# chonlei/neural-ode-ion-channels

Measured on AMD Instinct MI355X. Metric: trajectories/sec (sinewave protocol, 100k steps), higher is better.
Workload: dtype f64

## Files before the change

include/ionode.h:

```cpp
#ifndef IONODE_H
#define IONODE_H

#include <stddef.h>
#include <stdint.h>

#ifdef __cplusplus
extern "C" {
#endif

#define IONODE_ABI_VERSION 10

#define IONODE_MODEL_HH2 0
#define IONODE_MODEL_MARKOV6 1
#define IONODE_MODEL_NNF 2
#define IONODE_MODEL_NND 3

#define IONODE_STATUS_OK 0
#define IONODE_STATUS_DT_UNDERFLOW 1
#define IONODE_STATUS_NONFINITE 2
#define IONODE_STATUS_MAX_STEPS 3

#define IONODE_OK 0
#define IONODE_ERR_ARG (-1)
#define IONODE_ERR_UNSUPPORTED (-2)
// ... 25 lines not shown
  double t_eval_dt_hint;
  int64_t max_total_steps;
  double *ckpt;
  int32_t ckpt_cap;
  int32_t t_eval_exact;
  const double *sse_ref;
  double *sse_out;
  double max_step;
  const double *v_at_outputs;
  int64_t mlp_image_stride;
  int32_t traj_per_image;
  const int32_t *launch_order;
} ionode_desc;

#define IONODE_DEFAULT_MAX_TOTAL_STEPS 1000000

size_t ionode_mlp_packed_floats(int32_t mlp_layers, int32_t mlp_width);

int ionode_mlp_pack(const float *state_dict_flat, int32_t mlp_layers, int32_t mlp_width, float *packed);

int ionode_dopri5(const ionode_desc *d, const float *mlp_packed, const double *params, const double *prot_v,
                  const double *prot_t, const int32_t *prot_of_traj, const void *y0, const double *t_eval,
                  void *y_out, double *i_out, int32_t *status, int64_t *stats, void *stream);

int ionode_protocol_at_outputs(const ionode_desc *d, const double *prot_v, const double *prot_t, const double *t_eval,
                               double *v_out, void *stream);

int ionode_launch_geometry(const ionode_desc *d, int32_t out[4]);

const char *ionode_kernel_name(const ionode_desc *d);

const char *ionode_last_kernel_name(void);

int32_t ionode_lane_wise_from(int32_t model, int32_t mlp_width);

const char *ionode_last_error(void);
int32_t ionode_abi_version(void);


size_t ionode_grad_image_floats(int32_t mlp_layers, int32_t mlp_width);
int ionode_grad_pack(const float *state_dict_flat, int32_t mlp_layers, int32_t mlp_width, float *image);

size_t ionode_grad_record_floats(int32_t mlp_layers, int32_t mlp_width);

int ionode_dopri5_backward(const ionode_desc *d, int32_t it_begin, int32_t it_end, int32_t n_iter, const float *grad_image,
                           const double *params, const double *prot_v, const double *prot_t, const int32_t *prot_of_traj,
// ... 60 lines not shown
```

neural-ode-ion-channels_amd/capi.py:

```python
import ctypes as C
import os
import subprocess

import numpy as np
import torch

_HERE = os.path.dirname(os.path.abspath(__file__))
LIB_PATH = os.environ.get("IONODE_LIB") or os.path.join(_HERE, "libionode.so")

MODEL_HH2, MODEL_MARKOV6, MODEL_NNF, MODEL_NND = 0, 1, 2, 3
STATUS_OK, STATUS_DT_UNDERFLOW, STATUS_NONFINITE, STATUS_MAX_STEPS = 0, 1, 2, 3
STATUS_TEXT = {
    0: "ok",
    1: "underflow in dt",
    2: "non-finite values in state `y`",
    3: "max_num_steps exceeded",
}
ABI_VERSION = 10

EXPORTS = (
    "ionode_abi_version", "ionode_last_error", "ionode_mlp_packed_floats", "ionode_mlp_pack",
    "ionode_launch_geometry", "ionode_kernel_name", "ionode_last_kernel_name", "ionode_lane_wise_from", "ionode_dopri5", "ionode_protocol_at_outputs",
    "ionode_grad_image_floats", "ionode_grad_pack", "ionode_grad_record_floats", "ionode_dopri5_backward", "ionode_dopri5_backward_sse",
    "ionode_grad_packet_doubles", "ionode_dopri5_backward_recompute", "ionode_dopri5_backward_sweep",
    "ionode_dopri5_backward_sse_gc", "ionode_dopri5_backward_recompute_sse", "ionode_dopri5_backward_sweep_sse",
    "ionode_grad_partial_floats", "ionode_grad_reduce", "ionode_grad_reduce_unit", "ionode_grad_reduce_slabs", "ionode_grad_last_error",
    "ionode_regress_step", "ionode_adam_step", "ionode_image_refresh", "ionode_regress_plan",
)

SWEEP_BUFFERS = {
    "ionode_dopri5_backward": ("grad_image", "params", "prot_v", "prot_t", "prot_of_traj", "t_eval", "n_accepted", "grad_y", "state",
                               "records", "grad_params", "grad_y0"),
    "ionode_dopri5_backward_sse": ("params", "prot_v", "prot_t", "prot_of_traj", "t_eval", "n_accepted", "grad_sse", "state",
                                   "grad_params", "grad_y0"),
    "ionode_dopri5_backward_recompute": ("grad_image", "params", "prot_v", "prot_t", "prot_of_traj", "t_eval", "n_accepted", "grad_y",
                                         "records", "packets"),
    "ionode_dopri5_backward_sweep": ("grad_image", "params", "prot_v", "prot_t", "prot_of_traj", "t_eval", "n_accepted", "grad_y", "state",
                                     "records", "packets", "grad_params", "grad_y0"),
    "ionode_dopri5_backward_sse_gc": ("prot_v", "prot_t", "prot_of_traj", "t_eval", "n_accepted", "grad_sse", "packets", "sse_grad_y0"),
    "ionode_dopri5_backward_recompute_sse": ("grad_image", "params", "prot_v", "prot_t", "prot_of_traj", "t_eval", "n_accepted", "records",
                                             "packets"),
    "ionode_dopri5_backward_sweep_sse": ("grad_image", "params", "prot_v", "prot_t", "prot_of_traj", "t_eval", "n_accepted", "sse_grad_y0",
                                         "state", "records", "packets", "grad_params", "grad_y0"),
}


def n_state(model):
    return 6 if model == MODEL_MARKOV6 else 2


# ... 35 lines not shown

_lib = None


def lib():
    global _lib
    if _lib is None:
        if not os.path.exists(LIB_PATH):
            raise IonodeError(f"{LIB_PATH} is missing: run `python -c 'import __graft_entry__ as g; g.build()'` "
                              "(there is no CPU fallback for the integrator)")
        L = C.CDLL(LIB_PATH)
        L.ionode_abi_version.restype = C.c_int32
        L.ionode_last_error.restype = C.c_char_p
        L.ionode_kernel_name.restype = C.c_char_p
        L.ionode_kernel_name.argtypes = [C.POINTER(IonodeDesc)]
        L.ionode_mlp_packed_floats.restype = C.c_size_t
        L.ionode_mlp_packed_floats.argtypes = [C.c_int32, C.c_int32]
        L.ionode_mlp_pack.restype = C.c_int
        L.ionode_mlp_pack.argtypes = [C.c_void_p, C.c_int32, C.c_int32, C.c_void_p]
        L.ionode_launch_geometry.restype = C.c_int
        L.ionode_launch_geometry.argtypes = [C.POINTER(IonodeDesc), C.POINTER(C.c_int32 * 4)]
        L.ionode_dopri5.restype = C.c_int
        L.ionode_dopri5.argtypes = [C.POINTER(IonodeDesc)] + [C.c_void_p] * 12
        L.ionode_grad_last_error.restype = C.c_char_p
        for fn in (L.ionode_grad_image_floats, L.ionode_grad_record_floats, L.ionode_grad_partial_floats):
            fn.restype = C.c_size_t
            fn.argtypes = [C.c_int32, C.c_int32]
        L.ionode_grad_pack.restype = C.c_int
        L.ionode_grad_pack.argtypes = [C.c_void_p, C.c_int32, C.c_int32, C.c_void_p]
        L.ionode_grad_packet_doubles.restype = C.c_size_t
        L.ionode_grad_packet_doubles.argtypes = []
        for name, buffers in SWEEP_BUFFERS.items():
            getattr(L, name).restype = C.c_int
            getattr(L, name).argtypes = [C.POINTER(IonodeDesc), C.c_int32, C.c_int32, C.c_int32] + [C.c_void_p] * (len(buffers) + 1)
        L.ionode_grad_reduce.restype = C.c_int
        L.ionode_grad_reduce.argtypes = [C.c_int32, C.c_int32, C.c_void_p, C.c_int64, C.c_int32, C.c_void_p, C.c_void_p]
        L.ionode_grad_reduce_slabs.restype = C.c_int32
        L.ionode_grad_reduce_slabs.argtypes = [C.c_int32, C.c_int32, C.c_int64]
        L.ionode_grad_reduce_unit.restype = C.c_int
        L.ionode_grad_reduce_unit.argtypes = [C.c_int32, C.c_int32, C.c_void_p, C.c_int64, C.c_int32, C.c_void_p, C.c_void_p]
        L.ionode_regress_step.restype = C.c_int
        L.ionode_regress_step.argtypes = [C.c_int32, C.c_int32, C.c_void_p, C.c_void_p, C.c_void_p, C.c_void_p, C.c_int32,
                                          C.c_float, C.c_void_p, C.c_void_p, C.c_int32, C.c_void_p]
        L.ionode_regress_plan.restype = C.c_int
        L.ionode_regress_plan.argtypes = [C.c_int32, C.c_int32, C.POINTER(C.c_int32 * 3)]
        L.ionode_adam_step.restype = C.c_int
# ... 40 lines not shown
    return h.hexdigest()


def make_desc(**kw):
    d = IonodeDesc()
    for k, v in kw.items():
        setattr(d, k, v)
    return d


def launch_geometry(desc):
    out = (C.c_int32 * 4)()
    rc = lib().ionode_launch_geometry(C.byref(desc), C.byref(out))
    if rc != 0:
        raise IonodeError(last_error())
    return {"grid": out[0], "block": out[1], "lds_bytes": out[2], "tile_waves": out[3]}


def regress_plan(mlp_layers, mlp_width):
    out = (C.c_int32 * 3)()
    if lib().ionode_regress_plan(int(mlp_layers), int(mlp_width), C.byref(out)) != 0:
        raise IonodeError(lib().ionode_grad_last_error().decode())
    return {"generic": bool(out[0]), "wg_per_cu": out[1], "lds_bytes": out[2]}


def kernel_name(desc):
    return lib().ionode_kernel_name(C.byref(desc)).decode()


def _dev_ptr(t, dtype, name, shape=None):
    if t is None:
        return None
    if not isinstance(t, torch.Tensor) or not t.is_cuda:
        raise IonodeError(f"{name}: expected a CUDA/HIP tensor (the integrator has no CPU path)")
    if t.dtype != dtype or not t.is_contiguous():
        raise IonodeError(f"{name}: expected contiguous {dtype}, got {t.dtype} contiguous={t.is_contiguous()}")
    if shape is not None and tuple(t.shape) != tuple(shape):
        raise IonodeError(f"{name}: expected shape {tuple(shape)}, got {tuple(t.shape)}")
    return C.c_void_p(t.data_ptr())


_order_cache = {}


def _protocol_major(prot_of_traj):
    key = (prot_of_traj.data_ptr(), prot_of_traj._version, int(prot_of_traj.shape[0]), str(prot_of_traj.device))
# ... 78 lines not shown
        desc.sse_ref, desc.sse_out = sse_ref.data_ptr(), sse.data_ptr()
    elif not states:
        raise IonodeError("states=False needs sse_ref (something must be computed)")
    i_out = out.get("i")
    if current and i_out is None:
        i_out = torch.empty((B, Nt), dtype=torch.float64, device=dev)
    status = out.get("status")
    if status is None:
        status = torch.empty((B,), dtype=torch.int32, device=dev)
    st = out.get("stats")
    if stats and st is None:
        st = torch.empty((B, 4), dtype=torch.int64, device=dev)
    s = stream if stream is not None else torch.cuda.current_stream(dev).cuda_stream
    vtab = None
    if (current or sse_ref is not None) and model in (MODEL_HH2, MODEL_MARKOV6) and v_at_outputs is not None:
        if isinstance(v_at_outputs, str):
            if 4 * P <= B:
                vtab = protocol_at_outputs(desc, prot_v, prot_t, t_eval, stream=s)
        else:
            vtab = v_at_outputs
            _dev_ptr(vtab, torch.float64, "v_at_outputs", (P, Nt))
        if vtab is not None:
            desc.v_at_outputs = vtab.data_ptr()
    rc = lib().ionode_dopri5(
        C.byref(desc),
        _dev_ptr(mlp_packed, torch.float32, "mlp_packed"),
        _dev_ptr(params, torch.float64, "params", (B, params.shape[1])),
        _dev_ptr(prot_v, torch.float64, "prot_v"),
        _dev_ptr(prot_t, torch.float64, "prot_t", (Np,)) if prot_t is not None else None,
        _dev_ptr(prot_of_traj, torch.int32, "prot_of_traj", (B,)) if prot_of_traj is not None else None,
        _dev_ptr(y0, sdt, "y0"),
        _dev_ptr(t_eval, torch.float64, "t_eval"),
        _dev_ptr(y, sdt, "y_out", (B, Nt, D)) if y is not None else None,
        _dev_ptr(i_out, torch.float64, "i_out", (B, Nt)) if i_out is not None else None,
        _dev_ptr(status, torch.int32, "status", (B,)),
        _dev_ptr(st, torch.int64, "stats", (B, 4)) if st is not None else None,
        C.c_void_p(s),
    )
    if rc != 0:
        raise IonodeError(f"ionode_dopri5 failed ({rc}): {last_error()}")
    return {"y": y, "i": i_out, "status": status, "stats": st, "sse": sse, "desc": desc, "v_at_outputs": vtab,
            "kernel": lib().ionode_last_kernel_name().decode()}


def uniform_grid(t_eval):
    n = int(t_eval.shape[0])
    if n < 2:
        return None
    t0 = t_eval[0]
    dt = (t_eval[n - 1] - t0) / (n - 1)
    dev = (t_eval - (t0 + torch.arange(n, dtype=torch.float64, device=t_eval.device) * dt)).abs().max()
    t0, dt, dev = (float(x) for x in torch.stack([t0, dt, dev]).cpu())
    return (t0, dt, dev) if dt > 0 and dev <= 0.5 * dt else None


def sweep_launch(name, desc, it_begin, it_end, n_iter, stream, **buffers):
    names = SWEEP_BUFFERS[name]
    if set(buffers) != set(names):
        raise TypeError(f"{name}: missing {sorted(set(names) - set(buffers))}, unknown {sorted(set(buffers) - set(names))}")
    ptrs = [None if buffers[n] is None else C.c_void_p(buffers[n].data_ptr()) for n in names]
# ... 15 lines not shown
```

neural-ode-ion-channels_amd/csrc/ionode_attempt_body.hpp:

```cpp
#ifdef IONODE_STAMPS
    constexpr int NET = std::is_same<typename std::decay<decltype(IONODE_NET)>::type, MlpShrink4>::value ? 1 : 0;
    const unsigned long long att0_ = stamp_now();
#endif
    if constexpr (LW) {
#pragma unroll
      for (int i = 0; i < NPAR; ++i) asm volatile("" : "+v"(p[i]));
    }
    bool failed_now = false;
    if (active) {
      if ((int64_t)since >= a.max_steps || (int64_t)nacc + nrej >= a.max_total) { status = IONODE_STATUS_MAX_STEPS; failed_now = true; }
      else if (!(t + dt > t)) { status = IONODE_STATUS_DT_UNDERFLOW; failed_now = true; }
      else {
        bool fin = true;
#pragma unroll
        for (int d = 0; d < D; ++d) fin = fin && isfinite((double)y[d]);
        if (!fin) { status = IONODE_STATUS_NONFINITE; failed_now = true; }
      }
      if (failed_now) active = false;
    }
    {
      unsigned long long fm = __ballot(failed_now && lane < LPS);
      while (fm) {
        const int jj = __builtin_ctzll(fm);
        fm &= fm - 1;
// ... 140 lines not shown
      }
    }
    STAMP(stamps_, 8);
    if (LEAN || LEANM || a.te_dt > 0.0) {
      int n_out = 0;
      if (acc_now) {
        const double gf = floor((t1 - a.te_t0) * a.te_rdt);
        long long g = (gf < (double)(oi - 1)) ? (long long)(oi - 1) : ((gf > (double)(Nt - 1)) ? (long long)(Nt - 1) : (long long)gf);
        if ((LW && LEAN && D > 2) || (!LW && a.te_exact)) {
          while (g >= oi && te_at((int)g) > t1) --g;
          while (g + 1 < Nt && te_at((int)g + 1) <= t1) ++g;
        } else {
          while (g >= oi && a.t_eval[g] > t1) --g;
          while (g + 1 < Nt && a.t_eval[g + 1] <= t1) ++g;
        }
        n_out = (int)(g - oi + 1);
      }
      STAMP(stamps_, 9);
      if constexpr (!LW && G > 1) {
      constexpr int NS = (LPS >= WPS) ? LPS / WPS : 1;
      const bool exact = a.te_exact != 0;
      const bool want_i = (a.i_out != nullptr) || (a.sse_out != nullptr);
      const bool ugrid = a.prot_t == nullptr;
      int o_[NS], n_[NS], ip_[NS];
      double tk_[NS], plo_[NS], phi_[NS];
      bool inr_[NS];
      const double *pv_[NS];
#pragma unroll
      for (int k = 0; k < NS; ++k) {
        const int jj = wis + WPS * k;
        o_[k] = __builtin_amdgcn_readlane(oi, jj);
        n_[k] = (LPS >= WPS || jj < LPS) ? __builtin_amdgcn_readlane(n_out, jj) : 0;
        pv_[k] = a.prot_v + (size_t)__builtin_amdgcn_readlane(pidx, jj) * a.Np;
        tk_[k] = 0.0;
        if (lane < n_[k]) tk_[k] = exact ? te_at(o_[k] + lane) : a.t_eval[o_[k] + lane];
      }
      if (want_i && ugrid) {
#pragma unroll
        for (int k = 0; k < NS; ++k) {
          inr_[k] = protocol_index(a, tk_[k], ip_[k]);
          plo_[k] = pv_[k][ip_[k] - 1]; phi_[k] = pv_[k][ip_[k]];
        }
      }
      STAMP(stamps_, 10);
#pragma unroll
      for (int k = 0; k < NS; ++k) {
        const int jj = wis + WPS * k;
        const int n = n_[k], o = o_[k];
        if (n > 0) {
          const double t0b = bcast_f64(t0, jj), denb = bcast_f64(den, jj), rdenb = bcast_f64(rden, jj);
          S cb[5][D];
#pragma unroll
          for (int c = 0; c < 5; ++c)
#pragma unroll
            for (int d = 0; d < D; ++d) cb[c][d] = bcast<S>(ic[c][d], jj);
// ... 18 lines not shown
#pragma unroll
                for (int d = 0; d < D; ++d) out[d] = out[d] + xp * cb[c][d];
              }
              if (yo) store_state<S, D>(yo + (size_t)idx * D, out);
              if (want_i) {
                double vk;
                if (c0 == 0 && ugrid) vk = inr_[k] ? protocol_from(a, plo_[k], phi_[k], ip_[k], tk) : a.v_oob;
                else protocol_v(a, pv_[k], tk, vk);
                S gate;
                if (a.obs_open) gate = out[D - 1]; else gate = out[0] * out[1];
                if (a.obs_g != 1.0) gate = (S)a.obs_g * gate;
                const double ik = (double)gate * (vk - a.obs_e);
                if (io) io[idx] = ik;
                if (refb) { const double rr = ik - refb[idx]; sacc += rr * rr; }
              }
            }
          }
          if (a.sse_out) {
#pragma unroll
            for (int msk = 32; msk >= 1; msk >>= 1) sacc += __shfl_xor(sacc, msk);
            if (j == jj) sse += sacc;
          }
        }
      }
      oi += n_out;
      } else {
      bool packed_lane = false;
      if constexpr (LW && (VTAB || D > 2 || (CF2 && F::lean == Lean::States))) {
        constexpr int PK = 8, PKL = (D == 2) ? 4 : 2, NSL = PK / PKL;
        typedef S SV __attribute__((ext_vector_type(NSL)));
        const bool want_i = (a.i_out != nullptr) || (a.sse_out != nullptr);
        if (a.te_exact && (VTAB ? (want_i && (D > 2 || a.y_out == nullptr)) : (!want_i && a.y_out != nullptr))) {
          int lane_e = lane;
          asm volatile("" : "+v"(lane_e));
          packed_lane = n_out > 0 && lane_e < LPS && n_out <= 64;
          const unsigned long long emd = __ballot(packed_lane);
          auto emit_packed = [&](auto wi_tag) {
            constexpr bool WI = decltype(wi_tag)::value;
            const int nch = (n_out + PK - 1) / PK;
            if (packed_lane) *reinterpret_cast<int2 *>(lsm + lane_e * ROWB + 24) = make_int2(oi, oi + n_out);
            const int x = nch - 1;
            const unsigned long long m0 = __ballot(packed_lane && (x & 1)), m1 = __ballot(packed_lane && (x & 2)), m2 = __ballot(packed_lane && (x & 4));
            const int q = mbcnt(m0, mbcnt(emd)) + 2 * mbcnt(m1) + 4 * mbcnt(m2);
            const int C = __builtin_popcountll(emd) + __builtin_popcountll(m0) + 2 * __builtin_popcountll(m1) + 4 * __builtin_popcountll(m2);
#pragma unroll
            for (int i = 0; i < 8; ++i)
// ... 312 lines not shown
```

neural-ode-ion-channels_amd/csrc/ionode_capi.hip:

```cpp
#include <algorithm>
#include <cstdio>
#include <cstdlib>
#include <cstring>
#include <vector>

#include "ionode_launch.hpp"

namespace {

constexpr int kTile32From = 8192;
constexpr int kTile4Upto = 1024;
constexpr int kTile1Upto = 256;
constexpr int kTiny64From = 32769;
constexpr int kHh2LaneFrom = 49152;
constexpr int kMarkov6LaneFrom = 24576;

thread_local char g_err[256] = "";
thread_local const char *g_last_kernel = "";

void set_err(const char *fmt, const char *detail = "") { snprintf(g_err, sizeof g_err, fmt, detail); }

inline int np_of(int N) { return 16 * ((N + 15) / 16); }

struct Plan {
// ... 108 lines not shown
  if (!pl->v) {
    set_err("MLP width outside the compiled kernel variants: 1 <= N <= 512 (tuned tiles for N = 10, 100, 200, 500 -- architectures "
            "s00-s11 -- and the run-time-width tile for every other N; tile_waves must be 0 or 4 for the latter)");
    return IONODE_ERR_UNSUPPORTED;
  }
  const ionode::Variant *v = pl->v;
  const size_t tiles = (size_t)((d->n_traj + v->traj_per_tile - 1) / v->traj_per_tile);
  pl->grid = (unsigned)tiles;
  pl->block = 64u * v->G;
  pl->lds = v->lds_bytes(L, NT);
  if (v->shrink) {
    const char *ts = getenv("IONODE_TILE_SHRINK");
    pl->tile_shrink = ts == nullptr || ts[0] == '\0' || atoi(ts) != 0;
    pl->lds = std::max(pl->lds, ionode::MlpTile4::lds_bytes(L));
  }
  if (v->lane_wise) plan_lane_wise(pl, tiles, ((pl->lds + 15) & ~(size_t)15) + (size_t)ionode::LwLds::bytes(2, v->lds_key));
  if (d->traj_per_image > 0) {
    if (d->traj_per_image % v->traj_per_tile != 0 || d->mlp_image_stride < (int64_t)ionode_mlp_packed_floats(L, d->mlp_width)) {
      set_err("traj_per_image must be a multiple of the tile size (16; 64 with tile_waves = 64; 32 with tile_waves = 8) and mlp_image_stride at least one packed image");
      return IONODE_ERR_ARG;
    }
  }
  return IONODE_OK;
}

int make_plan(const ionode_desc *d, Plan *pl, bool want_current = false, bool explicit_grid = false) {
  if (!d) { set_err("null descriptor"); return IONODE_ERR_ARG; }
#ifdef IONODE_STAMPS
  const bool has_step_log = false;
#else
  const bool has_step_log = d->step_log != nullptr;
#endif
  const bool mlp = d->model == IONODE_MODEL_NNF || d->model == IONODE_MODEL_NND;
  const int D = d->model == IONODE_MODEL_MARKOV6 ? 6 : 2;
  if (d->model < 0 || d->model > 3) { set_err("unknown model"); return IONODE_ERR_ARG; }
  if (d->n_state != D) { set_err("n_state does not match model"); return IONODE_ERR_ARG; }
  if (d->n_traj < 1 || d->n_out < 1 || d->n_prot < 1 || d->prot_n < 2) { set_err("empty batch / grid / protocol"); return IONODE_ERR_ARG; }
  if (d->n_params < (D == 6 ? 12 : 8)) { set_err("n_params too small for model"); return IONODE_ERR_ARG; }
  if (!(d->rtol > 0) || !(d->atol >= 0) || !(d->prot_dt > 0)) { set_err("rtol/atol/prot_dt must be positive"); return IONODE_ERR_ARG; }
  const Ask k = {want_current, explicit_grid, has_step_log};
  return mlp ? plan_mlp(d, pl, k) : plan_closed(d, pl, k, D);
}

}

namespace ionode {
// ... 225 lines not shown
}

int ionode_launch_geometry(const ionode_desc *d, int32_t out[4]) {
  Plan pl;
  const int rc = make_plan(d, &pl);
  if (rc != IONODE_OK) return rc;
  out[0] = (int32_t)pl.grid;
  out[1] = (int32_t)pl.block;
  out[2] = (int32_t)pl.lds;
  out[3] = pl.v->G;
  return IONODE_OK;
}

const char *ionode_kernel_name(const ionode_desc *d) {
  Plan pl;
  if (make_plan(d, &pl, d && (d->sse_out != nullptr || d->v_at_outputs != nullptr)) != IONODE_OK) return "";
  return pl.v->name;
}

const char *ionode_last_kernel_name(void) { return g_last_kernel; }

int32_t ionode_lane_wise_from(int32_t model, int32_t mlp_width) { return lane_wise_from(model, mlp_width); }

int ionode_dopri5(const ionode_desc *d, const float *mlp_packed, const double *params, const double *prot_v,
                  const double *prot_t, const int32_t *prot_of_traj, const void *y0, const double *t_eval,
                  void *y_out, double *i_out, int32_t *status, int64_t *stats, void *stream) {
  Plan pl;
  const int rc = make_plan(d, &pl, i_out != nullptr || d->sse_out != nullptr, prot_t != nullptr);
  if (rc != IONODE_OK) return rc;
  const bool mlp = d->model == IONODE_MODEL_NNF || d->model == IONODE_MODEL_NND;
  if (!params || !prot_v || !y0 || !t_eval || (!y_out && !d->sse_out) || !status || (mlp && !mlp_packed)) {
    set_err("ionode_dopri5: required buffer is NULL");
    return IONODE_ERR_ARG;
  }
  if (d->sse_out && (!d->sse_ref || !(d->t_eval_dt_hint > 0.0) || d->n_out < 2)) {
    set_err("fused objective: sse_out needs sse_ref and the output-grid hint (t_eval_dt_hint > 0)");
    return IONODE_ERR_ARG;
  }
  ionode::KArgs a;
  memset(&a, 0, sizeof a);
  a.mlp = mlp_packed; a.params = params; a.prot_v = prot_v; a.prot_t = prot_t; a.prot_of_traj = prot_of_traj;
  a.y0 = y0; a.t_eval = t_eval; a.y_out = y_out; a.i_out = i_out; a.status = status; a.stats = stats;
  a.B = d->n_traj; a.Nt = d->n_out; a.P = d->n_prot; a.Np = d->prot_n; a.n_params = d->n_params;
  if (mlp) { a.L = d->mlp_layers; a.N = d->mlp_width; a.NP = np_of(d->mlp_width); a.NT = a.NP / 16; }
  a.max_steps = d->max_steps > 0 ? d->max_steps : (int64_t)2147483647;
  a.max_total = d->max_total_steps > 0 ? d->max_total_steps
                                       : (d->max_total_steps == 0 ? (int64_t)IONODE_DEFAULT_MAX_TOTAL_STEPS : INT64_MAX);
  a.ckpt = d->ckpt; a.ckpt_cap = d->ckpt ? d->ckpt_cap : 0;
  if (d->ckpt && d->ckpt_cap < 1) { set_err("ckpt given with ckpt_cap < 1"); return IONODE_ERR_ARG; }
  a.prot_rdt = 1.0 / d->prot_dt;
  a.dt_max = d->max_step > 0.0 ? d->max_step : __builtin_inf();
  a.prot_t0 = d->prot_t0; a.prot_dt = d->prot_dt; a.v_oob = d->v_oob; a.rtol = d->rtol; a.atol = d->atol;
  a.obs_g = d->obs_g; a.obs_e = d->obs_e; a.obs_open = d->obs_open_state_only;
  a.step_log = d->step_log; a.step_log_cap = d->step_log ? d->step_log_cap : 0;
  a.sse_ref = d->sse_ref; a.sse_out = d->sse_out; a.v_tab = d->v_at_outputs;
  if (mlp && d->traj_per_image > 0) { a.mlp_stride = d->mlp_image_stride; a.traj_per_img = d->traj_per_image; }
  if (d->launch_order) {
    if (a.traj_per_img > 0) { set_err("launch_order cannot be combined with traj_per_image (tiles of an image must stay together)"); return IONODE_ERR_ARG; }
    a.order = d->launch_order;
  }
  a.lw_bytes = (int32_t)pl.lw_bytes;
  a.te_t0 = d->t_eval_t0_hint; a.te_dt = (d->t_eval_dt_hint > 0.0 && d->n_out > 1) ? d->t_eval_dt_hint : 0.0;
  a.te_rdt = a.te_dt > 0.0 ? 1.0 / a.te_dt : 0.0;
  a.te_exact = (a.te_dt > 0.0 && d->t_eval_exact) ? 1 : 0;
  a.tile_shrink = pl.tile_shrink ? 1 : 0;
  const hipError_t e = pl.v->fn(a, pl.grid, pl.lds, reinterpret_cast<hipStream_t>(stream));
  if (e != hipSuccess) { set_err("kernel launch failed: %s", hipGetErrorString(e)); return IONODE_ERR_LAUNCH; }
  g_last_kernel = pl.v->name;
  return IONODE_OK;
}

int ionode_protocol_at_outputs(const ionode_desc *d, const double *prot_v, const double *prot_t, const double *t_eval,
                               double *v_out, void *stream) {
  if (!d || !prot_v || !t_eval || !v_out) { set_err("ionode_protocol_at_outputs: required buffer is NULL"); return IONODE_ERR_ARG; }
  if (d->n_out < 1 || d->n_prot < 1 || d->prot_n < 2 || !(d->prot_dt > 0)) { set_err("ionode_protocol_at_outputs: empty grid / protocol"); return IONODE_ERR_ARG; }
  ionode::KArgs a;
  memset(&a, 0, sizeof a);
  a.prot_v = prot_v; a.prot_t = prot_t; a.t_eval = t_eval; a.Nt = d->n_out; a.P = d->n_prot; a.Np = d->prot_n;
  a.prot_t0 = d->prot_t0; a.prot_dt = d->prot_dt; a.prot_rdt = 1.0 / d->prot_dt; a.v_oob = d->v_oob;
  const long long n = (long long)a.P * a.Nt;
  const unsigned grid = (unsigned)((n + 255) / 256 > 65536 ? 65536 : (n + 255) / 256);
  hipLaunchKernelGGL(ionode::ionode_protocol_at_outputs_kernel, dim3(grid), dim3(256), 0, reinterpret_cast<hipStream_t>(stream), a, v_out);
  const hipError_t e = hipGetLastError();
  if (e != hipSuccess) { set_err("kernel launch failed: %s", hipGetErrorString(e)); return IONODE_ERR_LAUNCH; }
  return IONODE_OK;
}

}
```

neural-ode-ion-channels_amd/csrc/ionode_device.hpp:

```cpp
#pragma once

#include <hip/hip_runtime.h>
#include <stdint.h>

#include <type_traits>

#include "../../include/ionode.h"
#include "ionode_form.hpp"
#include "ionode_kargs.hpp"
#include "ionode_math.hpp"

namespace ionode {

struct LwLds {
  static __host__ __device__ constexpr int rowb(int D) { return (4 + 5 * D) * 8; }
  static __host__ __device__ constexpr int aux_off(int D) { return 64 * rowb(D); }
  static __host__ __device__ constexpr int aux_bytes(int tail) { return (tail == 1 && IONODE_LEAN) ? 0 : 64 * 64; }
  static __host__ __device__ constexpr int owp_off(int D, int tail) { return aux_off(D) + aux_bytes(tail); }
  static __host__ __device__ constexpr int trl_off(int D, int tail) { return owp_off(D, tail) + 256; }
  static __host__ __device__ constexpr int clist_off(int D, int tail) { return trl_off(D, tail) + 256; }
  static __host__ __device__ constexpr int bytes(int D, int tail) { return clist_off(D, tail) + 1024; }
};
static_assert(LwLds::bytes(2, 1) <= 10240 && LwLds::bytes(2, 0) <= 12800 && LwLds::bytes(2, 2) <= 12800, "2-state kernels: 16 / 12 wavefronts per compute unit");

}

#include "ionode_mlp_tile.hpp"
#include "ionode_mlp_tile4.hpp"
#include "ionode_mlp_row1.hpp"
#include "ionode_mlp_lane.hpp"
#include "ionode_mlp_gen.hpp"
#include "ionode_rhs.hpp"

namespace ionode {

template <typename S, int D> __device__ __forceinline__ void store_state(S *dst, const S *v) {
  if constexpr (D == 2 && sizeof(S) == 8) {
    *reinterpret_cast<double2 *>(dst) = make_double2(v[0], v[1]);
  } else if constexpr (D == 2 && sizeof(S) == 4) {
    *reinterpret_cast<float2 *>(dst) = make_float2(v[0], v[1]);
  } else if constexpr (sizeof(S) == 8) {
#pragma unroll
    for (int d = 0; d < D; d += 2) *reinterpret_cast<double2 *>(dst + d) = make_double2(v[d], v[d + 1]);
  } else {
#pragma unroll
// ... 134 lines not shown
    if (a.y_out) store_state<S, D>(yout, y);
    if (iout) {
      double v0;
      protocol_v(a, pv, t, v0);
      S gate;
      if (a.obs_open) gate = y[D - 1]; else gate = y[0] * y[1];
      if (a.obs_g != 1.0) gate = (S)a.obs_g * gate;
      iout[0] = (double)gate * (v0 - a.obs_e);
    }
  }
  if (a.sse_out != nullptr && valid) {
    double v0;
    protocol_v(a, pv, t, v0);
    S gate;
    if (a.obs_open) gate = y[D - 1]; else gate = y[0] * y[1];
    if (a.obs_g != 1.0) gate = (S)a.obs_g * gate;
    const double r0 = (double)gate * (v0 - a.obs_e) - a.sse_ref[(size_t)pidx * Nt];
    sse = r0 * r0;
  }

  int oi = 1;
  int nacc = 0, nrej = 0;
  int since = 0;
  int status = IONODE_STATUS_OK;
  bool active = valid && Nt > 1;
  const S nan_s = (S)__builtin_nan("");

  double vst[5];
  bool inst[5];
  auto lookup_stages = [&](double tt, double dd) {
    const S tts = (S)tt, dds = (S)dd, tt1s = (S)(tt + dd);
    if (((MT::MLP && G > 1) || (!MT::MLP && (D > 2 || !VTAB))) && a.prot_t == nullptr) {
      double tq[5], lo[5], hi[5];
      int ix[5];
#pragma unroll
      for (int i = 0; i < 5; ++i) {
        tq[i] = (double)((i >= 4) ? R::prev_(tt1s) : tts + (S)kAlpha[i] * dds);
        inst[i] = protocol_index(a, tq[i], ix[i]);
      }
#pragma unroll
      for (int i = 0; i < 5; ++i) { lo[i] = pv[ix[i] - 1]; hi[i] = pv[ix[i]]; }
#pragma unroll
      for (int i = 0; i < 5; ++i) vst[i] = inst[i] ? protocol_from(a, lo[i], hi[i], ix[i], tq[i]) : a.v_oob;
      return;
    }
#pragma unroll
// ... 48 lines not shown
  if (threadIdx.x == 0 && a.step_log != nullptr) {
    if (blockIdx.x == 0 && a.step_log_cap >= 9) {
      a.step_log[32] = (double)att_cyc[0]; a.step_log[33] = (double)att_n[0];
      a.step_log[34] = (double)att_cyc[1]; a.step_log[35] = (double)att_n[1];
    }
    if (4 * a.step_log_cap >= 64 + (int64_t)gridDim.x) a.step_log[64 + blockIdx.x] = (double)att_n[1];
  }
#ifdef IONODE_ASM_STAMPS
  if constexpr (MT::MLP && G == 4 && NT == 13) {
    unsigned sv_;
    asm volatile("v_accvgpr_read_b32 %0, a92" : "=v"(sv_));
    if (blockIdx.x == 0 && threadIdx.x < 16 && a.step_log != nullptr && a.step_log_cap >= 8) a.step_log[16 + threadIdx.x] = (double)sv_;
  }
#endif
#endif
  if constexpr (LW) {
    if (a.sse_out != nullptr) {
#pragma unroll
      for (int m = 0; m < 8; ++m) sse += ssep[j * 8 + m];
    }
  }
  if (a.sse_out != nullptr && valid && lane < LPS && (WPS == 1 || (lane % WPS) == wis))
    a.sse_out[traj] = (status == IONODE_STATUS_OK) ? sse : __builtin_inf();
  if (valid && primary) {
    a.status[traj] = status;
    if (a.stats) {
      int64_t *st = a.stats + (size_t)traj * 4;
      st[0] = nacc;
      st[1] = nrej;
      st[2] = 2 + 6 * ((int64_t)nacc + nrej);
      st[3] = status;
    }
  }
}

}
```

neural-ode-ion-channels_amd/csrc/ionode_form.hpp:

```cpp
#pragma once

#include <type_traits>

#include "../../include/ionode.h"

#ifndef IONODE_LEAN
#define IONODE_LEAN 1
#endif
#ifndef IONODE_T64_WAVES
#define IONODE_T64_WAVES 1
#endif
#define IONODE_LW_TILES_PER_WG 4

namespace ionode {

template <int MODEL> struct ModelTraits {
  static constexpr int D = (MODEL == IONODE_MODEL_MARKOV6) ? 6 : 2;
  static constexpr int NPAR = (MODEL == IONODE_MODEL_MARKOV6) ? 12 : 8;
  static constexpr bool MLP = (MODEL == IONODE_MODEL_NNF || MODEL == IONODE_MODEL_NND);
};

template <int G, int RT, int NT, int PD, int NSETS> struct MlpTile;
struct MlpTile4;
template <int MRES_> struct MlpRow1T;
// ... 5 lines not shown

enum class Net { None, Tile, Tile4, Row1, Row1Deep, Lane, Gen };
enum class Lean { General, States, Table, Tile };

template <int MODEL, int G, int RT, int NT, int PD, int TAIL> struct KernelForm {
  static constexpr bool mlp = ModelTraits<MODEL>::MLP;
  static constexpr bool t64 = mlp && RT == 64;
  static constexpr bool lane_wise = !mlp || t64;
  static constexpr int nsets = (mlp && G > 1 && (TAIL & 4)) ? 2 : 1;
  static constexpr Net net = !mlp                                      ? Net::None
                             : (t64 && PD > 1)                         ? Net::Lane
                             : (G == 4 && NT == 13 && (TAIL & 32))     ? ((TAIL & 64) ? Net::Row1Deep : Net::Row1)
                             : (G == 4 && NT == 13 && (TAIL & 16))     ? Net::Tile4
                             : (G == 4 && NT == 0)                     ? Net::Gen
                                                                       : Net::Tile;
  static constexpr Lean lean = lane_wise ? (TAIL == 1 ? Lean::States : ((!mlp && TAIL == 2) ? Lean::Table : Lean::General))
                                         : ((G > 1 && (TAIL & 8)) ? Lean::Tile : Lean::General);
  static constexpr int lanes_per_set = !mlp ? (RT > 0 ? RT : 64) : t64 ? 64 : (net == Net::Row1 || net == Net::Row1Deep) ? 1 : net == Net::Tile4 ? 4 : 16;
  static constexpr int traj_per_tile = lanes_per_set * nsets;
  static constexpr int lds_key = lean == Lean::States ? 1 : (lean == Lean::Table ? 2 : 0);
  static constexpr int block_threads = 64 * (lane_wise ? IONODE_LW_TILES_PER_WG : G);
  static constexpr int waves_per_simd = t64 ? IONODE_T64_WAVES : (MODEL == IONODE_MODEL_HH2 ? 2 : 1);
  static constexpr bool shrink = net == Net::Tile && G == 4 && NT == 13 && PD == 13 && TAIL == 8;

  using Tile = MlpTile<G, (t64 ? 1 : (RT > 0 ? RT : 1)), (NT > 0 ? NT : 1), ((PD > 0 && net != Net::Lane) ? PD : 1), nsets>;
  using Mlp = std::conditional_t<net == Net::None, NoMlp,
              std::conditional_t<net == Net::Lane, MlpLane<(net == Net::Lane ? PD : 10)>,
              std::conditional_t<net == Net::Row1, MlpRow1,
              std::conditional_t<net == Net::Row1Deep, MlpRow1Deep,
              std::conditional_t<net == Net::Tile4, MlpTile4,
              std::conditional_t<net == Net::Gen, MlpGen, Tile>>>>>>;

  static_assert(mlp || G == 1, "closed-form models use one wavefront per tile");
  static_assert(!t64 || (G == 1 && NT == 1), "64 trajectories per wavefront is the resident-weights (N <= 16) path");
  static_assert(nsets == 1 || net == Net::Tile, "the 4- and one-trajectory tiles have one column set");
};

}
```

neural-ode-ion-channels_amd/csrc/ionode_kargs.hpp:

```cpp
#pragma once

#include <hip/hip_runtime.h>
#include <stdint.h>

#include "../../include/ionode.h"
#include "ionode_form.hpp"
#include "ionode_math.hpp"

namespace ionode {

struct KArgs {
  const float *mlp;
  const double *params;
  const double *prot_v;
  const double *prot_t;
  const int32_t *prot_of_traj;
  const void *y0;
  const double *t_eval;
  void *y_out;
  double *i_out;
  int32_t *status;
  int64_t *stats;
  int32_t B, Nt, P, Np, n_params, L, N, NP, NT;
  int64_t max_steps;
  int64_t max_total;
  double *ckpt;
  int32_t ckpt_cap;
  double prot_t0, prot_dt, v_oob, rtol, atol, obs_g, obs_e;
  double prot_rdt;
  double dt_max;
  int32_t obs_open;
  double *step_log;
  int64_t step_log_cap;
  const double *sse_ref;
  double *sse_out;
  double te_t0, te_dt;
  double te_rdt;
  int32_t te_exact;
  const double *v_tab;
  int64_t mlp_stride;
  int32_t traj_per_img;
  int32_t lw_bytes;
  const int32_t *order;
  int32_t tile_shrink;
};

__device__ __forceinline__ bool protocol_index(const KArgs &a, double t, int &i);
__device__ __forceinline__ double protocol_from(const KArgs &a, double v_lo, double v_hi, int i, double t);

__device__ __forceinline__ bool protocol_index(const KArgs &a, double t, int &i) {
  const int n = a.Np;
  const double t_last = a.prot_t0 + (double)(n - 1) * a.prot_dt;
  const bool inr = !(t < a.prot_t0 || t > t_last || t != t);
  const double u = div_by(t - a.prot_t0, a.prot_dt, a.prot_rdt);
  double ci = ceil(u);
  ci = (ci < 1.0) ? 1.0 : ci;
  ci = (ci > (double)(n - 1)) ? (double)(n - 1) : ci;
  i = inr ? (int)ci : 1;
  return inr;
}
__device__ __forceinline__ double protocol_from(const KArgs &a, double v_lo, double v_hi, int i, double t) {
  const double x_lo = a.prot_t0 + (double)(i - 1) * a.prot_dt;
  const double slope = div_by(v_hi - v_lo, a.prot_dt, a.prot_rdt);
  return slope * (t - x_lo) + v_lo;
}

__device__ __forceinline__ bool protocol_v(const KArgs &a, const double *__restrict__ pv, double t, double &v) {
// ... 22 lines not shown
```

neural-ode-ion-channels_amd/csrc/ionode_launch.hpp:

```cpp
#pragma once
#include "ionode_device.hpp"

namespace ionode {

using LaunchFn = hipError_t (*)(const KArgs &, unsigned grid, size_t lds, hipStream_t);

struct Variant {
  int model, f32;
  int G;
  int NT;
  Net net;
  Lean lean;
  int traj_per_tile;
  int lds_key;
  bool lane_wise, shrink;
  size_t (*lds_bytes)(int L, int NT);
  LaunchFn fn;
  const char *name;
};

template <typename F> size_t net_lds_bytes(int L, int NT) {
  if constexpr (F::net == Net::None) return 0;
  else if constexpr (F::net == Net::Gen) return F::Mlp::lds_bytes(L, NT);
  else if constexpr (F::net == Net::Tile) return F::Mlp::lds_total(L);
  else return F::Mlp::lds_bytes(L);
}

template <int MODEL, typename S, int G, int RT, int NT, int PD, int TAIL>
hipError_t launch(const KArgs &a, unsigned grid, size_t lds, hipStream_t s) {
  using F = KernelForm<MODEL, G, RT, NT, PD, TAIL>;
  auto kern = ionode_dopri5_kernel<MODEL, S, G, RT, NT, PD, TAIL>;
  if constexpr (F::lane_wise) {
    const size_t need = (size_t)LwLds::bytes(ModelTraits<MODEL>::D, F::lds_key);
    if ((size_t)a.lw_bytes < need || (a.lw_bytes & 15) || lds < (size_t)IONODE_LW_TILES_PER_WG * (size_t)a.lw_bytes) return hipErrorInvalidValue;
  }
  if (lds > 64 * 1024) {
    hipError_t e = hipFuncSetAttribute(reinterpret_cast<const void *>(kern),
                                       hipFuncAttributeMaxDynamicSharedMemorySize, (int)lds);
    if (e != hipSuccess) return e;
  }
  hipLaunchKernelGGL(kern, dim3(grid), dim3(F::block_threads), lds, s, a);
  return hipGetLastError();
}

template <int MODEL, typename S, int F32, int G, int RT, int NT, int PD, int TAIL>
constexpr Variant make_variant(const char *name) {
  using F = KernelForm<MODEL, G, RT, NT, PD, TAIL>;
  return Variant{MODEL, F32, G, NT, F::net, F::lean, F::traj_per_tile, F::lds_key, F::lane_wise, F::shrink, &net_lds_bytes<F>,
                 &launch<MODEL, S, G, RT, NT, PD, TAIL>, name};
}

#define IONODE_VARIANT(MODEL, S, F32, G, RT, NT, PD, TAIL) IONODE_VARIANT_(MODEL, S, F32, G, RT, NT, PD, TAIL)
#define IONODE_VARIANT_(MODEL, S, F32, G, RT, NT, PD, TAIL) \
  make_variant<MODEL, S, F32, G, RT, NT, PD, TAIL>("ionode_dopri5_kernel<" #MODEL ", " #S ", " #G ", " #RT ", " #NT ", " #PD ", " #TAIL ">")
#define IONODE_MLP_VARIANTS(MODEL, S, F32)                                                      \
  IONODE_VARIANT(MODEL, S, F32, 1, 1, 1, 1, 0), IONODE_VARIANT(MODEL, S, F32, 4, 4, 7, 7, 0),        \
       \
      IONODE_VARIANT(MODEL, S, F32, 1, 64, 1, 1, 0), IONODE_VARIANT(MODEL, S, F32, 1, 64, 1, 1, 1),      \
            \
      IONODE_VARIANT(MODEL, S, F32, 1, 64, 1, 10, 0), IONODE_VARIANT(MODEL, S, F32, 1, 64, 1, 10, 1),    \
      IONODE_VARIANT(MODEL, S, F32, 4, 4, 13, 13, 0), IONODE_VARIANT(MODEL, S, F32, 4, 8, 32, 4, 0),     \
       \
      IONODE_VARIANT(MODEL, S, F32, 4, 4, 13, 13, 4),                                                     \
       \
      IONODE_VARIANT(MODEL, S, F32, 4, 4, 13, 13, 8), IONODE_VARIANT(MODEL, S, F32, 4, 4, 13, 13, 12),    \
       \
      IONODE_VARIANT(MODEL, S, F32, 4, 4, 13, 13, 16), IONODE_VARIANT(MODEL, S, F32, 4, 4, 13, 13, 24),   \
       \
      IONODE_VARIANT(MODEL, S, F32, 4, 4, 13, 13, 32), IONODE_VARIANT(MODEL, S, F32, 4, 4, 13, 13, 40),   \
       \
      IONODE_VARIANT(MODEL, S, F32, 4, 4, 13, 13, 96), IONODE_VARIANT(MODEL, S, F32, 4, 4, 13, 13, 104),  \
// ... 13 lines not shown
```

Measured before the change: 12370.

## Defer dense output interpolation to a separate expand kernel via compact step records

Instead of evaluating the dense-output polynomial and writing every output sample inside the integrator kernel, the integrator now stores one compact record per accepted step (t0, denominator, cursor, interpolation coefficients) into a workspace. A second kernel expands those records into y_out and i_out in parallel afterwards, falling back to inline emission once the per-trajectory record capacity is exhausted. The aim is to take the scattered output writes and interpolation work out of the latency-bound integrator loop. The cost is an extra workspace, an extra kernel launch, and record writes from the integrator. It applies only to the shrink tile variant with two states and no SSE output.

Measured after the change: 12570 (median of 6 runs). 1.02x the previous value.

```diff
diff --git a/include/ionode.h b/include/ionode.h
--- a/include/ionode.h
+++ b/include/ionode.h
@@ -71,6 +71,12 @@
 int ionode_dopri5(const ionode_desc *d, const float *mlp_packed, const double *params, const double *prot_v,
                   const double *prot_t, const int32_t *prot_of_traj, const void *y0, const double *t_eval,
                   void *y_out, double *i_out, int32_t *status, int64_t *stats, void *stream);
+
+int ionode_dense_defer_plan(const ionode_desc *d, int32_t want_current, int64_t out[2]);
+int ionode_dopri5_deferred(const ionode_desc *d, const float *mlp_packed, const double *params, const double *prot_v,
+                           const double *prot_t, const int32_t *prot_of_traj, const void *y0, const double *t_eval,
+                           void *y_out, double *i_out, int32_t *status, int64_t *stats, void *stream, void *workspace,
+                           int64_t workspace_bytes);
 
 int ionode_protocol_at_outputs(const ionode_desc *d, const double *prot_v, const double *prot_t, const double *t_eval,
                                double *v_out, void *stream);
diff --git a/neural-ode-ion-channels_amd/capi.py b/neural-ode-ion-channels_amd/capi.py
--- a/neural-ode-ion-channels_amd/capi.py
+++ b/neural-ode-ion-channels_amd/capi.py
@@ -26,6 +26,7 @@
     "ionode_dopri5_backward_sse_gc", "ionode_dopri5_backward_recompute_sse", "ionode_dopri5_backward_sweep_sse",
     "ionode_grad_partial_floats", "ionode_grad_reduce", "ionode_grad_reduce_unit", "ionode_grad_reduce_slabs", "ionode_grad_last_error",
     "ionode_regress_step", "ionode_adam_step", "ionode_image_refresh", "ionode_regress_plan",
+    "ionode_dense_defer_plan", "ionode_dopri5_deferred",
 )
 
 SWEEP_BUFFERS = {
@@ -107,6 +108,10 @@
         L.ionode_launch_geometry.argtypes = [C.POINTER(IonodeDesc), C.POINTER(C.c_int32 * 4)]
         L.ionode_dopri5.restype = C.c_int
         L.ionode_dopri5.argtypes = [C.POINTER(IonodeDesc)] + [C.c_void_p] * 12
+        L.ionode_dopri5_deferred.restype = C.c_int
+        L.ionode_dopri5_deferred.argtypes = [C.POINTER(IonodeDesc)] + [C.c_void_p] * 13 + [C.c_int64]
+        L.ionode_dense_defer_plan.restype = C.c_int
+        L.ionode_dense_defer_plan.argtypes = [C.POINTER(IonodeDesc), C.c_int32, C.POINTER(C.c_int64 * 2)]
         L.ionode_grad_last_error.restype = C.c_char_p
         for fn in (L.ionode_grad_image_floats, L.ionode_grad_record_floats, L.ionode_grad_partial_floats):
             fn.restype = C.c_size_t
@@ -193,6 +198,13 @@
     if lib().ionode_regress_plan(int(mlp_layers), int(mlp_width), C.byref(out)) != 0:
         raise IonodeError(lib().ionode_grad_last_error().decode())
     return {"generic": bool(out[0]), "wg_per_cu": out[1], "lds_bytes": out[2]}
+
+
+def dense_defer_plan(desc, want_current):
+    out = (C.c_int64 * 2)()
+    if lib().ionode_dense_defer_plan(C.byref(desc), int(bool(want_current)), C.byref(out)) != 0:
+        raise IonodeError(last_error())
+    return {"capacity": int(out[0]), "workspace_bytes": int(out[1])}
 
 
 def kernel_name(desc):
@@ -317,7 +329,12 @@
             _dev_ptr(vtab, torch.float64, "v_at_outputs", (P, Nt))
         if vtab is not None:
             desc.v_at_outputs = vtab.data_ptr()
-    rc = lib().ionode_dopri5(
+    ws = None
+    if stream is None and prot_t is None and y is not None:
+        plan = dense_defer_plan(desc, i_out is not None)
+        if plan["capacity"] > 0:
+            ws = torch.empty((plan["workspace_bytes"],), dtype=torch.uint8, device=dev)
+    rc = lib().ionode_dopri5_deferred(
         C.byref(desc),
         _dev_ptr(mlp_packed, torch.float32, "mlp_packed"),
         _dev_ptr(params, torch.float64, "params", (B, params.shape[1])),
@@ -331,6 +348,8 @@
         _dev_ptr(status, torch.int32, "status", (B,)),
         _dev_ptr(st, torch.int64, "stats", (B, 4)) if st is not None else None,
         C.c_void_p(s),
+        C.c_void_p(ws.data_ptr()) if ws is not None else None,
+        ws.numel() if ws is not None else 0,
     )
     if rc != 0:
         raise IonodeError(f"ionode_dopri5 failed ({rc}): {last_error()}")
diff --git a/neural-ode-ion-channels_amd/csrc/ionode_attempt_body.hpp b/neural-ode-ion-channels_amd/csrc/ionode_attempt_body.hpp
--- a/neural-ode-ion-channels_amd/csrc/ionode_attempt_body.hpp
+++ b/neural-ode-ion-channels_amd/csrc/ionode_attempt_body.hpp
@@ -186,6 +186,37 @@
       const bool exact = a.te_exact != 0;
       const bool want_i = (a.i_out != nullptr) || (a.sse_out != nullptr);
       const bool ugrid = a.prot_t == nullptr;
+      int n_emit = n_out;
+      if constexpr (F::defer) {
+        if (a.defer_rec != nullptr) {
+          using Rec = DenseRecord<D>;
+          const bool rec_now = n_out > 0 && nrec < a.defer_cap;
+          const int rq = lane >> 4;
+          auto chunk = [&](int r) {
+            if (r == 0) return make_double2(t0, den);
+            if (r == 1) return make_double2(rden, Rec::pack_cursor(oi_before, n_out));
+            const int e = 2 * (r - 2);
+            return make_double2((double)ic[e / D][e % D], (double)ic[(e + 1) / D][(e + 1) % D]);
+          };
+          double2 *__restrict__ row = reinterpret_cast<double2 *>(a.defer_rec + ((size_t)traj * (size_t)a.defer_cap + (size_t)nrec) * Rec::ROW);
+#pragma unroll
+          for (int w = 0; 4 * w < Rec::CHUNKS; ++w) {
+            if (wis == w) {
+              double2 v = chunk(4 * w);
+#pragma unroll
+              for (int qq = 1; qq < 4; ++qq) {
+                if (4 * w + qq < Rec::CHUNKS) {
+                  const double2 c = chunk(4 * w + qq);
+                  if (rq == qq) v = c;
+                }
+              }
+              if (rec_now && 4 * w + rq < Rec::CHUNKS) row[4 * w + rq] = v;
+            }
+          }
+          if (rec_now) { n_emit = 0; ++nrec; }
+        }
+      }
+      if (!F::defer || __ballot(n_emit > 0) != 0ull) {
       int o_[NS], n_[NS], ip_[NS];
       double tk_[NS], plo_[NS], phi_[NS];
       bool inr_[NS];
@@ -194,7 +225,7 @@
       for (int k = 0; k < NS; ++k) {
         const int jj = wis + WPS * k;
         o_[k] = __builtin_amdgcn_readlane(oi, jj);
-        n_[k] = (LPS >= WPS || jj < LPS) ? __builtin_amdgcn_readlane(n_out, jj) : 0;
+        n_[k] = (LPS >= WPS || jj < LPS) ? __builtin_amdgcn_readlane(n_emit, jj) : 0;
         pv_[k] = a.prot_v + (size_t)__builtin_amdgcn_readlane(pidx, jj) * a.Np;
         tk_[k] = 0.0;
         if (lane < n_[k]) tk_[k] = exact ? te_at(o_[k] + lane) : a.t_eval[o_[k] + lane];
@@ -259,6 +290,7 @@
             if (j == jj) sse += sacc;
           }
         }
+      }
       }
       oi += n_out;
       } else {
diff --git a/neural-ode-ion-channels_amd/csrc/ionode_capi.hip b/neural-ode-ion-channels_amd/csrc/ionode_capi.hip
--- a/neural-ode-ion-channels_amd/csrc/ionode_capi.hip
+++ b/neural-ode-ion-channels_amd/csrc/ionode_capi.hip
@@ -154,6 +154,30 @@
     }
   }
   return IONODE_OK;
+}
+
+struct DeferPlan {
+  int64_t cap = 0, bytes = 0;
+};
+DeferPlan plan_defer(const ionode_desc *d, const Plan &pl, bool want_i) {
+  DeferPlan p;
+  if (!pl.v->defer || d->sse_out != nullptr || d->n_state != 2) return p;
+  const char *sw = getenv("IONODE_DEFER_DENSE");
+  if (sw != nullptr && sw[0] != '\0' && atoi(sw) == 0) return p;
+  using Rec = ionode::DenseRecord<2>;
+  const int64_t B = d->n_traj, Nt = d->n_out;
+  const char *fc = getenv("IONODE_DEFER_DENSE_CAP");
+  int64_t cap = (fc != nullptr && fc[0] != '\0') ? atoll(fc) : 0;
+  const bool forced = cap > 0;
+  if (!forced) {
+    const int64_t out_bytes = B * Nt * 2 * (d->state_f32 ? 4 : 8) + (want_i ? B * Nt * 8 : 0);
+    cap = (out_bytes / 4) / (B * Rec::BYTES);
+  }
+  cap = std::min<int64_t>(cap, Nt - 1);
+  if (cap < (forced ? 1 : 64)) return p;
+  p.cap = cap;
+  p.bytes = (int64_t)Rec::workspace_bytes(B, cap);
+  return p;
 }
 
 int make_plan(const ionode_desc *d, Plan *pl, bool want_current = false, bool explicit_grid = false) {
@@ -425,9 +449,23 @@
 
 int32_t ionode_lane_wise_from(int32_t model, int32_t mlp_width) { return lane_wise_from(model, mlp_width); }
 
-int ionode_dopri5(const ionode_desc *d, const float *mlp_packed, const double *params, const double *prot_v,
-                  const double *prot_t, const int32_t *prot_of_traj, const void *y0, const double *t_eval,
-                  void *y_out, double *i_out, int32_t *status, int64_t *stats, void *stream) {
+int ionode_dense_defer_plan(const ionode_desc *d, int32_t want_current, int64_t out[2]) {
+  Plan pl;
+  const int rc = make_plan(d, &pl, want_current != 0 || (d && d->sse_out != nullptr));
+  if (rc != IONODE_OK) return rc;
+  const DeferPlan dp = plan_defer(d, pl, want_current != 0);
+  out[0] = dp.cap;
+  out[1] = dp.bytes;
+  return IONODE_OK;
+}
+
+}
+
+namespace {
+
+int dopri5_impl(const ionode_desc *d, const float *mlp_packed, const double *params, const double *prot_v,
+                const double *prot_t, const int32_t *prot_of_traj, const void *y0, const double *t_eval,
+                void *y_out, double *i_out, int32_t *status, int64_t *stats, void *stream, void *workspace, int64_t workspace_bytes) {
   Plan pl;
   const int rc = make_plan(d, &pl, i_out != nullptr || d->sse_out != nullptr, prot_t != nullptr);
   if (rc != IONODE_OK) return rc;
@@ -467,10 +505,47 @@
   a.te_rdt = a.te_dt > 0.0 ? 1.0 / a.te_dt : 0.0;
   a.te_exact = (a.te_dt > 0.0 && d->t_eval_exact) ? 1 : 0;
   a.tile_shrink = pl.tile_shrink ? 1 : 0;
-  const hipError_t e = pl.v->fn(a, pl.grid, pl.lds, reinterpret_cast<hipStream_t>(stream));
+  DeferPlan dp;
+  if (workspace != nullptr && prot_t == nullptr && y_out != nullptr) dp = plan_defer(d, pl, i_out != nullptr);
+  if (dp.cap > 0) {
+    if (workspace_bytes < dp.bytes || (reinterpret_cast<uintptr_t>(workspace) & 15) != 0) {
+      set_err("ionode_dopri5_deferred: workspace smaller than ionode_dense_defer_plan() asks for, or not 16-byte aligned");
+      return IONODE_ERR_ARG;
+    }
+    a.defer_count = static_cast<int32_t *>(workspace);
+    a.defer_rec = reinterpret_cast<double *>(static_cast<unsigned char *>(workspace) + ionode::DenseRecord<2>::records_offset(d->n_traj));
+    a.defer_cap = (int32_t)dp.cap;
+  }
+  hipError_t e = pl.v->fn(a, pl.grid, pl.lds, reinterpret_cast<hipStream_t>(stream));
   if (e != hipSuccess) { set_err("kernel launch failed: %s", hipGetErrorString(e)); return IONODE_ERR_LAUNCH; }
+  if (dp.cap > 0) {
+    const dim3 grid((unsigned)std::min<int64_t>((dp.cap + ionode::kExpandRecordsPerWg - 1) / ionode::kExpandRecordsPerWg, ionode::kExpandMaxBlocks),
+                    (unsigned)std::min(d->n_traj, 65535));
+    if (d->state_f32) hipLaunchKernelGGL((ionode::ionode_dense_expand_kernel<float, 2>), grid, dim3(256), 0, reinterpret_cast<hipStream_t>(stream), a);
+    else hipLaunchKernelGGL((ionode::ionode_dense_expand_kernel<double, 2>), grid, dim3(256), 0, reinterpret_cast<hipStream_t>(stream), a);
+    e = hipGetLastError();
+    if (e != hipSuccess) { set_err("kernel launch failed: %s", hipGetErrorString(e)); return IONODE_ERR_LAUNCH; }
+  }
   g_last_kernel = pl.v->name;
   return IONODE_OK;
+}
+
+}
+
+extern "C" {
+
+int ionode_dopri5(const ionode_desc *d, const float *mlp_packed, const double *params, const double *prot_v,
+                  const double *prot_t, const int32_t *prot_of_traj, const void *y0, const double *t_eval,
+                  void *y_out, double *i_out, int32_t *status, int64_t *stats, void *stream) {
+  return dopri5_impl(d, mlp_packed, params, prot_v, prot_t, prot_of_traj, y0, t_eval, y_out, i_out, status, stats, stream, nullptr, 0);
+}
+
+int ionode_dopri5_deferred(const ionode_desc *d, const float *mlp_packed, const double *params, const double *prot_v,
+                           const double *prot_t, const int32_t *prot_of_traj, const void *y0, const double *t_eval,
+                           void *y_out, double *i_out, int32_t *status, int64_t *stats, void *stream, void *workspace,
+                           int64_t workspace_bytes) {
+  return dopri5_impl(d, mlp_packed, params, prot_v, prot_t, prot_of_traj, y0, t_eval, y_out, i_out, status, stats, stream, workspace,
+                     workspace_bytes);
 }
 
 int ionode_protocol_at_outputs(const ionode_desc *d, const double *prot_v, const double *prot_t, const double *t_eval,
diff --git a/neural-ode-ion-channels_amd/csrc/ionode_dense_expand.hpp b/neural-ode-ion-channels_amd/csrc/ionode_dense_expand.hpp
--- /dev/null
+++ b/neural-ode-ion-channels_amd/csrc/ionode_dense_expand.hpp
@@ -0,0 +1,94 @@
+#pragma once
+
+#include <hip/hip_runtime.h>
+#include <stdint.h>
+
+#include "ionode_kargs.hpp"
+#include "ionode_math.hpp"
+
+namespace ionode {
+
+template <int D> struct DenseRecord {
+  static constexpr int ROW = 4 + 5 * D;
+  static constexpr int BYTES = ROW * 8;
+  static constexpr int CHUNKS = ROW / 2;
+  static constexpr int T0 = 0, DEN = 1, RDEN = 2, CURSOR = 3, COEF = 4;
+  static_assert(ROW % 2 == 0, "records are whole 16-byte chunks");
+  static __host__ __device__ constexpr size_t records_offset(int64_t B) { return ((size_t)B * 4 + 15) & ~(size_t)15; }
+  static __host__ __device__ constexpr size_t workspace_bytes(int64_t B, int64_t cap) { return records_offset(B) + (size_t)B * (size_t)cap * BYTES; }
+  static __device__ __forceinline__ double pack_cursor(int oi_before, int n_out) { return __hiloint2double(n_out, oi_before); }
+  static __device__ __forceinline__ int cursor_oi(double w) { return __double2loint(w); }
+  static __device__ __forceinline__ int cursor_n(double w) { return __double2hiint(w); }
+};
+
+constexpr int kExpandRecordsPerWg = 16;
+constexpr int kExpandMaxBlocks = 128;
+
+template <typename S, int D> __global__ void __launch_bounds__(256) ionode_dense_expand_kernel(const KArgs a) {
+  using Rec = DenseRecord<D>;
+  const int lane = threadIdx.x & 63;
+  const int wv = __builtin_amdgcn_readfirstlane(threadIdx.x >> 6);
+  const int Nt = a.Nt;
+  auto te_at = [&](int idx) -> double { return a.te_t0 + (double)idx * a.te_dt; };
+  const bool want_i = a.i_out != nullptr;
+  for (int tr = (int)blockIdx.y; tr < a.B; tr += (int)gridDim.y) {
+    int cnt = a.defer_count[tr];
+    cnt = cnt < a.defer_cap ? cnt : a.defer_cap;
+    if ((int)blockIdx.x * kExpandRecordsPerWg >= cnt) continue;
+    const int pj = a.prot_of_traj ? a.prot_of_traj[tr] : (tr % a.P);
+    const double *__restrict__ pv = a.prot_v + (size_t)pj * a.Np;
+    S *__restrict__ yo = a.y_out ? reinterpret_cast<S *>(a.y_out) + (size_t)tr * Nt * D : nullptr;
+    double *__restrict__ io = a.i_out ? a.i_out + (size_t)tr * Nt : nullptr;
+    for (int r0 = (int)blockIdx.x * kExpandRecordsPerWg; r0 < cnt; r0 += (int)gridDim.x * kExpandRecordsPerWg) {
+    const int r1 = (r0 + kExpandRecordsPerWg < cnt) ? r0 + kExpandRecordsPerWg : cnt;
+    for (int ri = r0 + wv; ri < r1; ri += 4) {
+      const double *__restrict__ rec = a.defer_rec + ((size_t)tr * (size_t)a.defer_cap + (size_t)ri) * Rec::ROW;
+      const double t0b = rec[Rec::T0], denb = rec[Rec::DEN], rdenb = rec[Rec::RDEN];
+      const double cur = rec[Rec::CURSOR];
+      const int o = Rec::cursor_oi(cur), n = Rec::cursor_n(cur);
+      S cb[5][D];
+#pragma unroll
+      for (int c = 0; c < 5; ++c)
+#pragma unroll
+        for (int d = 0; d < D; ++d) cb[c][d] = (S)rec[Rec::COEF + c * D + d];
+      for (int c0 = 0; c0 < n; c0 += 64) {
+        const int idx = o + c0 + lane;
+        if (c0 + lane < n && idx < Nt) {
+          const double tk = te_at(idx);
+          const S x = (S)div_pos(tk - t0b, denb, rdenb);
+          S out[D];
+          S xp = x;
+#pragma unroll
+          for (int d = 0; d < D; ++d) out[d] = cb[0][d] + x * cb[1][d];
+#pragma unroll
+          for (int c = 2; c < 5; ++c) {
+            xp = xp * x;
+#pragma unroll
+            for (int d = 0; d < D; ++d) out[d] = out[d] + xp * cb[c][d];
+          }
+          if (yo) {
+            if constexpr (sizeof(S) == 8) {
+#pragma unroll
+              for (int d = 0; d < D; d += 2) *reinterpret_cast<double2 *>(yo + (size_t)idx * D + d) = make_double2(out[d], out[d + 1]);
+            } else {
+#pragma unroll
+              for (int d = 0; d < D; d += 2) *reinterpret_cast<float2 *>(yo + (size_t)idx * D + d) = make_float2(out[d], out[d + 1]);
+            }
+          }
+          if (want_i) {
+            int ip;
+            const bool inr = protocol_index(a, tk, ip);
+            const double vk = inr ? protocol_from(a, pv[ip - 1], pv[ip], ip, tk) : a.v_oob;
+            S gate;
+            if (a.obs_open) gate = out[D - 1]; else gate = out[0] * out[1];
+            if (a.obs_g != 1.0) gate = (S)a.obs_g * gate;
+            io[idx] = (double)gate * (vk - a.obs_e);
+          }
+        }
+      }
+    }
+    }
+  }
+}
+
+}
diff --git a/neural-ode-ion-channels_amd/csrc/ionode_device.hpp b/neural-ode-ion-channels_amd/csrc/ionode_device.hpp
--- a/neural-ode-ion-channels_amd/csrc/ionode_device.hpp
+++ b/neural-ode-ion-channels_amd/csrc/ionode_device.hpp
@@ -9,6 +9,7 @@
 #include "ionode_form.hpp"
 #include "ionode_kargs.hpp"
 #include "ionode_math.hpp"
+#include "ionode_dense_expand.hpp"
 
 namespace ionode {
 
@@ -21,6 +22,7 @@
   static __host__ __device__ constexpr int clist_off(int D, int tail) { return trl_off(D, tail) + 256; }
   static __host__ __device__ constexpr int bytes(int D, int tail) { return clist_off(D, tail) + 1024; }
 };
+static_assert(LwLds::rowb(2) == DenseRecord<2>::BYTES && LwLds::rowb(6) == DenseRecord<6>::BYTES, "the deferred-output record is the lane-wise kernels' row");
 static_assert(LwLds::bytes(2, 1) <= 10240 && LwLds::bytes(2, 0) <= 12800 && LwLds::bytes(2, 2) <= 12800, "2-state kernels: 16 / 12 wavefronts per compute unit");
 
 }
@@ -201,6 +203,7 @@
   int oi = 1;
   int nacc = 0, nrej = 0;
   int since = 0;
+  [[maybe_unused]] int nrec = 0;
   int status = IONODE_STATUS_OK;
   bool active = valid && Nt > 1;
   const S nan_s = (S)__builtin_nan("");
@@ -295,6 +298,9 @@
   }
   if (a.sse_out != nullptr && valid && lane < LPS && (WPS == 1 || (lane % WPS) == wis))
     a.sse_out[traj] = (status == IONODE_STATUS_OK) ? sse : __builtin_inf();
+  if constexpr (F::defer) {
+    if (a.defer_rec != nullptr && valid && primary) a.defer_count[traj] = nrec;
+  }
   if (valid && primary) {
     a.status[traj] = status;
     if (a.stats) {
diff --git a/neural-ode-ion-channels_amd/csrc/ionode_form.hpp b/neural-ode-ion-channels_amd/csrc/ionode_form.hpp
--- a/neural-ode-ion-channels_amd/csrc/ionode_form.hpp
+++ b/neural-ode-ion-channels_amd/csrc/ionode_form.hpp
@@ -51,6 +51,7 @@
   static constexpr int block_threads = 64 * (lane_wise ? IONODE_LW_TILES_PER_WG : G);
   static constexpr int waves_per_simd = t64 ? IONODE_T64_WAVES : (MODEL == IONODE_MODEL_HH2 ? 2 : 1);
   static constexpr bool shrink = net == Net::Tile && G == 4 && NT == 13 && PD == 13 && TAIL == 8;
+  static constexpr bool defer = shrink;
 
   using Tile = MlpTile<G, (t64 ? 1 : (RT > 0 ? RT : 1)), (NT > 0 ? NT : 1), ((PD > 0 && net != Net::Lane) ? PD : 1), nsets>;
   using Mlp = std::conditional_t<net == Net::None, NoMlp,
diff --git a/neural-ode-ion-channels_amd/csrc/ionode_kargs.hpp b/neural-ode-ion-channels_amd/csrc/ionode_kargs.hpp
--- a/neural-ode-ion-channels_amd/csrc/ionode_kargs.hpp
+++ b/neural-ode-ion-channels_amd/csrc/ionode_kargs.hpp
@@ -43,6 +43,9 @@
   int32_t lw_bytes;
   const int32_t *order;
   int32_t tile_shrink;
+  int32_t *defer_count;
+  double *defer_rec;
+  int32_t defer_cap;
 };
 
 __device__ __forceinline__ bool protocol_index(const KArgs &a, double t, int &i);
diff --git a/neural-ode-ion-channels_amd/csrc/ionode_launch.hpp b/neural-ode-ion-channels_amd/csrc/ionode_launch.hpp
--- a/neural-ode-ion-channels_amd/csrc/ionode_launch.hpp
+++ b/neural-ode-ion-channels_amd/csrc/ionode_launch.hpp
@@ -14,6 +14,7 @@
   int traj_per_tile;
   int lds_key;
   bool lane_wise, shrink;
+  bool defer;
   size_t (*lds_bytes)(int L, int NT);
   LaunchFn fn;
   const char *name;
@@ -46,7 +47,7 @@
 template <int MODEL, typename S, int F32, int G, int RT, int NT, int PD, int TAIL>
 constexpr Variant make_variant(const char *name) {
   using F = KernelForm<MODEL, G, RT, NT, PD, TAIL>;
-  return Variant{MODEL, F32, G, NT, F::net, F::lean, F::traj_per_tile, F::lds_key, F::lane_wise, F::shrink, &net_lds_bytes<F>,
+  return Variant{MODEL, F32, G, NT, F::net, F::lean, F::traj_per_tile, F::lds_key, F::lane_wise, F::shrink, F::defer, &net_lds_bytes<F>,
                  &launch<MODEL, S, G, RT, NT, PD, TAIL>, name};
 }
 
```
